# TravisDai/DLRM-FlexFlow

Hardware: AMD Instinct MI355X
Metric: samples/sec DLRM (MLPerf-like) at 1/2/4/8 MI355X; SOAP speedup vs pure DP (higher is better)
Workload: dtype fp32; 1 GPU; global_batch=8192, seq_len=1, parallelism=dp1, tables_rows=187767399, embedding_dim=128, interaction=dot, hip_graph=True, backend=none, process_world=1, fp32_gemm=bf16x3-split-big+native-f32-mfma, gemm_tuned_entries=21, gemm_staging=lds-dma

## Files before the change

csrc/bindings/hip_ops.cpp:

```cpp
#include <torch/extension.h>
#include <ATen/hip/HIPContext.h>
#include <cstring>
#include <vector>

extern "C" {
void fm_sgd_update_segs(float* W, float* G, float* V, unsigned short* Wc, const float* lr, const long* off,
                        const long* len, int nseg, float wd, float mom, int nesterov, int zero_g, hipStream_t s);
void fm_image_normalize(const unsigned char* src, void* dst, long N, int H, int W, const float* mean, const float* stdv,
                        int bf16, hipStream_t s);
int fm_gemm_dw_sgd(const void* A, long lda, const void* B, long ldb, float* W, long ldw, unsigned short* Wc, float* V,
                   const float* lr, float wd, float mom, int nesterov, int M, int N, int K, float* ws, long ws_bytes,
                   float* rowsum_a, int cfg, hipStream_t stream);
int fm_gemm_f32_dw_sgd(const float* A, long lda, const float* B, long ldb, float* W, long ldw, unsigned short* Wc,
                       float* V, const float* lr, float wd, float mom, int nesterov, int M, int N, int K, float* ws,
                       long ws_bytes, float* rowsum_a, int cfg, hipStream_t stream);
int fm_gemm(const void* A, long lda, long sA, int a_kcontig, const void* B, long ldb, long sB, int b_kcontig, void* C,
            long ldc, long sC, int c_fp32, const float* bias, int M, int N, int K, int batch, float alpha, int beta,
            int act, float* ws, long ws_bytes, int ksplit_req, const void* act_y, long lday, int bwd_act,
            float* colsum, float* rowsum_a, hipStream_t stream);
void fm_gemm_f32_set_split(int on);
void fm_gemm_set_dma(int on);
int fm_gemm_dma_enabled();
void fm_embedding_set_bwd_mode(int count);
int fm_gemm_f32_get_split();
// ... 9 lines not shown
                        int nesterov, int bf16, hipStream_t s);
void fm_skinny_fwd_f32_launch(const float* x, long ldx, const float* w, const float* bias, float* y, long ldy, long B, int K,
                              int act, hipStream_t s);
void fm_skinny_bwd_f32_launch(const float* x, long ldx, const float* w, const float* y, long ldy, const float* dy, long lddy,
                              float* dx, long lddx, int dx_acc, float* dw, float* db, long B, int K, int act, int bact,
                              hipStream_t s);
void fm_skinny_fwd(const void* x, long ldx, const void* w, const float* bias, void* y, long ldy, long B, int K, int act,
                   hipStream_t s);
void fm_skinny_bwd(const void* x, long ldx, const void* w, const void* y, long ldy, const void* dy, long lddy, void* dx,
                   long lddx, int dx_acc, float* dw, float* db, long B, int K, int act, int bact, hipStream_t s);
void fm_init_fill(float* out, long rows, long cols, long r0, long c0, long ldg, int kind, unsigned seed, float a, float b,
                  hipStream_t s);
void fm_embedding_fwd(const void* idx, int idx64, const float* W, void* out, int out_bf16, long B, int bag, int rows, int D,
                      long ldo, float scale, hipStream_t s);
void fm_embedding_bwd(const void* idx, int idx64, const void* dy, int dy_bf16, float* W, const float* lr, long B, int bag,
                      int rows, int D, long ldg, float scale, hipStream_t s);
void fm_embedding_fwd_multi(int n, const float* const* W, const void* const* idx, const int* idx64, void* const* out,
                            const long* ldo, const long* lo, const int* rows, const int* D, const int* bag,
                            const float* scale, int out_bf16, long B, hipStream_t st);
void fm_embedding_bwd_multi(int n, float* const* W, const void* const* idx, const int* idx64, const void* const* dy,
                            const long* ldg, const long* lo, const int* rows, const int* D, const int* bag,
                            const float* scale, int dy_bf16, const float* lr, long B, int* const* owner,
                            int* const* dups, int* const* ndup, hipStream_t st);
void fm_sdp_coalesce(int n, const void* const* idx, const int* idx64, const void* const* dy, const long* ldg,
                     const long* lo, const int* rows, const int* D, const int* bag, const float* scale, int dy_bf16, long B,
                     int* const* slot, int* const* cid, int* const* ids, float* const* g, int* const* count, hipStream_t st);
void fm_sdp_apply_segments(int n, int segs, int own_seg, float* const* W, const int* D, const int* const* seg_ids,
                           const float* const* seg_g, const int* const* seg_count, int* const* slot, int* const* own_count,
                           const int* nmax, const float* lr, hipStream_t st);
void fm_emb_adagrad_apply(int n, float* const* W, float* const* H, const int* D, const int* const* ids,
                          const float* const* g, int* const* count, int* const* slot, const int* nmax, const float* lr,
                          float eps, hipStream_t st);
void fm_emb_rowwise_adagrad_apply(int n, float* const* W, float* const* h, const int* D, const int* const* ids,
                                  const float* const* g, int* const* count, int* const* slot, const int* nmax,
                                  const float* lr, float eps, hipStream_t st);
void fm_sdp_rowwise_merge_segments(int n, int segs, const int* rows, const int* D, const int* const* seg_ids,
                                   const float* const* seg_g, const int* const* seg_count, const int* const* own_ids,
                                   int* const* own_count, int* const* slot, int* const* mids, float* const* mg,
                                   int* const* mcount, const int* nmax, const int* mcap, hipStream_t st);
void fm_strided_copy4_run(const void* src, void* dst, int bf16, const int* d, const long* ss, const long* ts, long so,
                          long to, int acc, hipStream_t st);
void fm_dot_interaction_fwd(const void* const* z, int F, long ldz, void* out, long ldo, long B, int D, int W, int self,
                            hipStream_t s);
void fm_dot_interaction_bwd(const void* const* z, int F, long ldz, const void* dout, long ldo, void* const* dz, long lddz,
                            unsigned acc_mask, long B, int D, int self, hipStream_t s);
void fm_dot_interaction_fwd_f32(const float* const* z, int F, long ldz, float* out, long ldo, long B, int D, int W, int self,
// ... 388 lines not shown
  bool any = false;
  if (claim.has_value()) {
    TORCH_CHECK(claim->size() == 3 * W.size(), "claim: 3 buffers per table");
    for (size_t k = 0; k < W.size(); ++k) {
      const auto& o = (*claim)[3 * k];
      if (!o.has_value() || !o->defined()) continue;
      const auto& d = (*claim)[3 * k + 1];
      const auto& c = (*claim)[3 * k + 2];
      TORCH_CHECK(o->scalar_type() == torch::kInt32 && o->numel() >= W[k].size(0), "claim owner: int32 [rows]");
      TORCH_CHECK(d.has_value() && d->scalar_type() == torch::kInt32 && d->numel() >= idx[k].numel(), "claim dups");
      TORCH_CHECK(c.has_value() && c->scalar_type() == torch::kInt32 && c->numel() >= 1, "claim ndup");
      own[k] = o->data_ptr<int>();
      dup[k] = d->data_ptr<int>();
      nd[k] = c->data_ptr<int>();
      any = true;
    }
  }
  fm_embedding_bwd_multi((int)W.size(), a.Wm.data(), a.idx.data(), a.idx64.data(), a.cact.data(), a.ld.data(), lo.data(),
                         a.rows.data(), a.D.data(), a.bag.data(), a.scale.data(), is_bf16(dy[0]),
                         lr.has_value() && lr->defined() ? lr->data_ptr<float>() : nullptr, a.B,
                         any ? own.data() : nullptr, any ? dup.data() : nullptr, any ? nd.data() : nullptr, cur());
}

void sdp_coalesce(std::vector<torch::Tensor> W, std::vector<torch::Tensor> idx, std::vector<torch::Tensor> dy,
                  std::vector<int64_t> ldg, std::vector<double> scale, std::vector<int64_t> row_lo,
                  std::vector<torch::Tensor> slot, std::vector<torch::Tensor> cid, std::vector<torch::Tensor> ids,
                  std::vector<torch::Tensor> g, std::vector<torch::Tensor> count) {
  if (W.empty()) return;
  TabArgs a = tab_args(W, idx, dy, ldg, scale);
  std::vector<long> lo = row_offsets(row_lo, W.size());
  const size_t n = W.size();
  TORCH_CHECK(slot.size() == n && cid.size() == n && ids.size() == n && g.size() == n && count.size() == n,
              "sdp_coalesce: one buffer of each kind per table");
  std::vector<int*> ps, pc, pi, pn;
  std::vector<float*> pg;
  for (size_t k = 0; k < n; ++k) {
    TORCH_CHECK(slot[k].scalar_type() == torch::kInt32 && slot[k].numel() >= W[k].size(0), "sdp slot: int32 [rows]");
    TORCH_CHECK(cid[k].scalar_type() == torch::kInt32 && cid[k].numel() >= idx[k].numel(), "sdp cid: int32 [B*bag]");
    TORCH_CHECK(ids[k].scalar_type() == torch::kInt32 && ids[k].numel() >= idx[k].numel(), "sdp ids: int32 [B*bag]");
    TORCH_CHECK(g[k].scalar_type() == torch::kFloat32 && g[k].numel() >= idx[k].numel() * W[k].size(1),
                "sdp g: fp32 [B*bag, D]");
    TORCH_CHECK(count[k].scalar_type() == torch::kInt32 && count[k].numel() >= 1, "sdp count: int32 [1]");
    ps.push_back(slot[k].data_ptr<int>());
    pc.push_back(cid[k].data_ptr<int>());
    pi.push_back(ids[k].data_ptr<int>());
    pg.push_back(g[k].data_ptr<float>());
// ... 869 lines not shown
  m.def("cnhwc_wprep", &cnhwc_wprep);
  m.def("conv_nhwc_fwd", &conv_nhwc_fwd);
  m.def("conv_nhwc_dgrad", &conv_nhwc_dgrad);
  m.def("gemm_f32_set_split", [](int mode) { fm_gemm_f32_set_split(mode); });
  m.def("gemm_set_dma", [](int on) { fm_gemm_set_dma(on); });
  m.def("gemm_dma_enabled", []() { return fm_gemm_dma_enabled(); });
  m.def("gemm_f32_get_split", []() { return fm_gemm_f32_get_split(); });
  m.def("embedding_set_bwd_mode", [](bool count) { fm_embedding_set_bwd_mode(count ? 1 : 0); });
  m.def("conv_nhwc_dgrad_strided", &conv_nhwc_dgrad_strided);
  m.def("conv_nhwc_wgrad", &conv_nhwc_wgrad);
  m.def("conv_s2d", &conv_s2d);
  m.def("stem_supported", &stem_supported);
  m.def("stem_wgrad_ws", &stem_wgrad_ws);
  m.def("stem_wf_elems", &stem_wf_elems);
  m.def("stem_fwd", &stem_fwd);
  m.def("stem_wgrad", &stem_wgrad);
  m.def("conv_w_s2d", &conv_w_s2d);
  m.def("embedding_fwd", &embedding_fwd);
  m.def("embedding_bwd", &embedding_bwd);
  m.def("embedding_fwd_multi", &embedding_fwd_multi, py::arg("W"), py::arg("idx"), py::arg("out"), py::arg("ldo"),
        py::arg("scale"), py::arg("row_lo") = std::vector<int64_t>{});
  m.def("embedding_bwd_multi", &embedding_bwd_multi, py::arg("W"), py::arg("idx"), py::arg("dy"), py::arg("ldg"),
        py::arg("scale"), py::arg("lr"), py::arg("claim"), py::arg("row_lo") = std::vector<int64_t>{});
  m.def("strided_copy4", &strided_copy4);
  m.def("sdp_coalesce", &sdp_coalesce);
  m.def("sdp_apply", &sdp_apply);
  m.def("emb_adagrad_apply", &emb_adagrad_apply);
  m.def("emb_rowwise_adagrad_apply", &emb_rowwise_adagrad_apply);
  m.def("sdp_rowwise_merge", &sdp_rowwise_merge);
  m.def("dot_fwd", &dot_fwd);
  m.def("dot_bwd", &dot_bwd, py::arg("zs"), py::arg("ldz"), py::arg("dout"), py::arg("ldo"), py::arg("dzs"),
        py::arg("lddz"), py::arg("acc_mask"), py::arg("D"), py::arg("self"), py::arg("act0") = 10);
  m.def("sgd", &sgd);
  m.def("adam", &adam);
  m.def("adagrad", &adagrad);
  m.def("cast_bf16", &cast_bf16);
  m.def("loss", &loss, py::arg("loss_type"), py::arg("logits"), py::arg("labels"), py::arg("grad"), py::arg("scale"),
        py::arg("acc"), py::arg("mask"), py::arg("clamp_t") = 0.0);
  m.def("unary_fwd", &unary_fwd);
  m.def("unary_bwd", &unary_bwd);
  m.def("binary_fwd", &binary_fwd);
  m.def("binary_bwd", &binary_bwd);
  m.def("act_bwd_bias", &act_bwd_bias);
  m.def("multi_copy", &multi_copy);
  m.def("image_normalize", &image_normalize);
  m.def("permute", &permute);
// ... 18 lines not shown
```

csrc/cpu/cpu_ops.cc:

```cpp
#include <torch/extension.h>
#include <ATen/Parallel.h>

#include <algorithm>
#include <cstdint>

#include "emb_kernels.h"

namespace {

void use_aten_pool() {
  static const bool done = [] {
    flexmi::cpu::set_parallel_for([](int64_t n, int64_t grain, int64_t max_threads,
                                     const std::function<void(int64_t, int64_t)>& fn) {
      if (max_threads > 0 && max_threads <= n) grain = std::max<int64_t>(grain, (n + max_threads - 1) / max_threads);
      at::parallel_for(0, n, grain, [&](int64_t b, int64_t e) { fn(b, e); });
    });
    return true;
  }();
  (void)done;
}

void check(const torch::Tensor& W, const torch::Tensor& idx, const torch::Tensor& rowt, const char* what) {
  TORCH_CHECK(W.device().is_cpu() && idx.device().is_cpu() && rowt.device().is_cpu(), what, ": CPU tensors");
  TORCH_CHECK(W.scalar_type() == torch::kFloat32 && W.dim() == 2 && W.is_contiguous(), what, ": contiguous fp32 table [R,D]");
  TORCH_CHECK(idx.dim() == 2 && idx.is_contiguous() &&
                  (idx.scalar_type() == torch::kInt32 || idx.scalar_type() == torch::kInt64), what,
              ": contiguous int32/int64 indices [B,bag]");
  TORCH_CHECK(rowt.scalar_type() == torch::kFloat32 && rowt.dim() == 2 && rowt.size(0) == idx.size(0) &&
// ... 6 lines not shown
  if (idx.scalar_type() == torch::kInt32)
    flexmi::cpu::embedding_bag_forward<int32_t>(W.data_ptr<float>(), W.size(0), W.size(1), idx.data_ptr<int32_t>(),
                                                idx.size(0), idx.size(1), row_lo, (float)scale, out.data_ptr<float>(),
                                                out.stride(0));
  else
    flexmi::cpu::embedding_bag_forward<int64_t>(W.data_ptr<float>(), W.size(0), W.size(1), idx.data_ptr<int64_t>(),
                                                idx.size(0), idx.size(1), row_lo, (float)scale, out.data_ptr<float>(),
                                                out.stride(0));
}

void embedding_bwd(torch::Tensor target, torch::Tensor idx, torch::Tensor dy, int64_t row_lo, double alpha) {
  check(target, idx, dy, "embedding_bwd");
  use_aten_pool();
  const int64_t B = idx.size(0), bag = idx.size(1), D = target.size(1);
  const int workers = (int)std::max<int64_t>(1, std::min<int64_t>(at::get_num_threads(), (B * bag * D) / 16384 + 1));
  if (idx.scalar_type() == torch::kInt32)
    flexmi::cpu::embedding_bag_backward<int32_t>(target.data_ptr<float>(), target.size(0), D, idx.data_ptr<int32_t>(), B,
                                                 bag, row_lo, dy.data_ptr<float>(), dy.stride(0), (float)alpha, workers);
  else
    flexmi::cpu::embedding_bag_backward<int64_t>(target.data_ptr<float>(), target.size(0), D, idx.data_ptr<int64_t>(), B,
                                                 bag, row_lo, dy.data_ptr<float>(), dy.stride(0), (float)alpha, workers);
}

bool avx2() { return flexmi::cpu::has_avx2(); }

}

void register_init_metrics(pybind11::module& m);

PYBIND11_MODULE(_cpu, m) {
  m.doc() = "flexmi native CPU kernels (embedding bag forward / backward / fused sparse SGD, counter-based init, loss + metrics)";
  m.def("embedding_fwd", &embedding_fwd, "out = scale * bag-sum of table rows");
  m.def("embedding_bwd", &embedding_bwd, "table rows += alpha * dy (dense grad or fused SGD)");
  m.def("avx2", &avx2);
  register_init_metrics(m);
}
```

csrc/cpu/emb_kernels.cc:

```cpp
#include "emb_kernels.h"

#include <immintrin.h>

#include <algorithm>
#include <thread>
#include <vector>

namespace flexmi {
namespace cpu {

namespace {

ParallelFor g_pf;

void default_parallel_for(int64_t n, int64_t grain, int64_t max_threads, const std::function<void(int64_t, int64_t)>& fn) {
  const int64_t hw = std::max<int64_t>(1, (int64_t)std::thread::hardware_concurrency());
  const int64_t nt = std::max<int64_t>(1, std::min<int64_t>({hw, max_threads > 0 ? max_threads : hw, (n + grain - 1) / grain}));
  if (nt <= 1) {
    fn(0, n);
    return;
  }
  std::vector<std::thread> th;
  const int64_t per = (n + nt - 1) / nt;
  for (int64_t t = 0; t < nt; ++t) {
// ... 91 lines not shown
  pfor(B, std::max<int64_t>(1, 2048 / std::max<int64_t>(1, D * bag / 64)), 0, [&](int64_t b0, int64_t b1) {
    for (int64_t b = b0; b < b1; ++b) {
      if (avx) bag_avx2<I>(W, rows, D, idx + b * bag, bag, row_lo, scale, out + b * ld_out);
      else bag_scalar<I>(W, rows, D, idx + b * bag, bag, row_lo, scale, out + b * ld_out);
    }
  });
}

template <typename I>
void embedding_bag_backward(float* target, int64_t rows, int64_t D, const I* idx, int64_t B, int64_t bag, int64_t row_lo,
                            const float* dy, int64_t ld_dy, float alpha, int workers) {
  const int64_t nw = std::max<int64_t>(1, workers > 0 ? workers : (B * bag * D) / 16384 + 1);
  pfor(nw, 1, nw, [&](int64_t p0, int64_t p1) {
    for (int64_t p = p0; p < p1; ++p)
      for (int64_t b = 0; b < B; ++b)
        for (int64_t j = 0; j < bag; ++j) {
          const int64_t r = (int64_t)idx[b * bag + j] - row_lo;
          if (r < 0 || r >= rows || r % nw != p) continue;
          axpy(target + r * D, dy + b * ld_dy, alpha, D);
        }
  });
}

template void embedding_bag_forward<int32_t>(const float*, int64_t, int64_t, const int32_t*, int64_t, int64_t, int64_t, float,
                                             float*, int64_t);
template void embedding_bag_forward<int64_t>(const float*, int64_t, int64_t, const int64_t*, int64_t, int64_t, int64_t, float,
                                             float*, int64_t);
template void embedding_bag_backward<int32_t>(float*, int64_t, int64_t, const int32_t*, int64_t, int64_t, int64_t,
                                              const float*, int64_t, float, int);
template void embedding_bag_backward<int64_t>(float*, int64_t, int64_t, const int64_t*, int64_t, int64_t, int64_t,
                                              const float*, int64_t, float, int);

}
}
```

csrc/cpu/emb_kernels.h:

```cpp
#pragma once
#include <cstdint>
#include <functional>

namespace flexmi {
namespace cpu {

using ParallelFor = std::function<void(int64_t, int64_t, int64_t, const std::function<void(int64_t, int64_t)>&)>;
void set_parallel_for(ParallelFor pf);

bool has_avx2();

template <typename I>
void embedding_bag_forward(const float* W, int64_t rows, int64_t D, const I* idx, int64_t B, int64_t bag, int64_t row_lo,
                           float scale, float* out, int64_t ld_out);

template <typename I>
void embedding_bag_backward(float* target, int64_t rows, int64_t D, const I* idx, int64_t B, int64_t bag, int64_t row_lo,
                            const float* dy, int64_t ld_dy, float alpha, int workers);

}
}
```

csrc/kernels/embedding.hip:

```cpp
#include "common.h"

#include <algorithm>
#include <cstdlib>
#include <cstring>
#include <vector>

namespace {

constexpr int MAXT = 32;
constexpr int TINY_ROWS = 16;

struct TabDesc {
  const float* W;
  const void* idx;
  void* act;
  long ld;
  long lo;
  int rows, D, bag;
  float scale;
};

FM_DEVICE long local_row(long r, long lo, int rows, bool& ok) {
  const long l = r - lo;
  ok = (unsigned long)l < (unsigned long)rows;
// ... 425 lines not shown

template <bool I64>
void launch_bwd(const TabSet& s, int m, bool tiny, bool dy_bf16, const float* lr, long B, int maxD, hipStream_t st) {
  if (tiny) {
    size_t lds = 0;
    for (int i = 0; i < m; ++i) lds = std::max(lds, (size_t)s.t[i].rows * s.t[i].D * 4 * 4);
    static bool attr = false;
    if (!attr) {
      (void)hipFuncSetAttribute((const void*)fm_emb_bwd_tiny_multi<unsigned short, I64>,
                                hipFuncAttributeMaxDynamicSharedMemorySize, 160 << 10);
      (void)hipFuncSetAttribute((const void*)fm_emb_bwd_tiny_multi<float, I64>,
                                hipFuncAttributeMaxDynamicSharedMemorySize, 160 << 10);
      attr = true;
    }
    const int chunk = B <= 16384 ? 64 : B <= 32768 ? 128 : 256;
    dim3 grid((unsigned)((B + chunk - 1) / chunk), m);
    if (dy_bf16) hipLaunchKernelGGL((fm_emb_bwd_tiny_multi<unsigned short, I64>), grid, dim3(256), lds, st, s, lr, B, chunk);
    else hipLaunchKernelGGL((fm_emb_bwd_tiny_multi<float, I64>), grid, dim3(256), lds, st, s, lr, B, chunk);
  } else {
    const int rpi = std::max(1, 256 / std::min(256, maxD));
    dim3 grid((unsigned)std::max<long>(1, emb_bwd_cap(std::min<long>((B + rpi - 1) / rpi, 2048))), m);
    if (dy_bf16) hipLaunchKernelGGL((fm_emb_bwd_atomic_multi<unsigned short, I64>), grid, dim3(256), 0, st, s, lr, B);
    else hipLaunchKernelGGL((fm_emb_bwd_atomic_multi<float, I64>), grid, dim3(256), 0, st, s, lr, B);
  }
}

struct SdpDesc {
  const void* idx;
  const void* dy;
  long ld;
  long lo;
  int rows, D, bag;
  float scale;
  int* slot;
  int* cid;
  int* ids;
  float* g;
  int* count;
};
struct SdpSet {
  SdpDesc t[MAXT];
  int n;
};

template <bool I64>
__global__ void __launch_bounds__(256) fm_sdp_claim(SdpSet s, long B) {
// ... 393 lines not shown
    for (int k = 0; k < n; ++k) {
      if (claimable(k)) continue;
      if (kind_of(k) == kind && (idx64[k] != 0) == wide) sel.push_back(k);
    }
    for (size_t base = 0; base < sel.size(); base += MAXT) {
      TabSet s;
      int m = (int)std::min<size_t>(MAXT, sel.size() - base);
      int maxD = 1;
      for (int i = 0; i < m; ++i) {
        int k = sel[base + i];
        s.t[i] = TabDesc{W[k], idx[k], const_cast<void*>(dy[k]), ldg[k], lo ? lo[k] : 0, rows[k], D[k], bag[k], scale[k]};
        maxD = std::max(maxD, D[k]);
      }
      s.n = m;
      if (wide) {
        launch_bwd<true>(s, m, tiny, dy_bf16, lr, B, maxD, st);
      } else {
        launch_bwd<false>(s, m, tiny, dy_bf16, lr, B, maxD, st);
      }
    }
  }
}

extern "C" void fm_embedding_fwd(const void* idx, int idx64, const float* W, void* out, int out_bf16, long B, int bag,
                                 int rows, int D, long ldo, float scale, hipStream_t s) {
  fm_embedding_fwd_multi(1, &W, &idx, &idx64, &out, &ldo, nullptr, &rows, &D, &bag, &scale, out_bf16, B, s);
}

extern "C" void fm_embedding_bwd(const void* idx, int idx64, const void* dy, int dy_bf16, float* W, const float* lr,
                                 long B, int bag, int rows, int D, long ldg, float scale, hipStream_t s) {
  fm_embedding_bwd_multi(1, &W, &idx, &idx64, &dy, &ldg, nullptr, &rows, &D, &bag, &scale, dy_bf16, lr, B, nullptr,
                         nullptr, nullptr, s);
}

extern "C" void fm_sdp_coalesce(int n, const void* const* idx, const int* idx64, const void* const* dy, const long* ldg,
                                const long* lo, const int* rows, const int* D, const int* bag, const float* scale,
                                int dy_bf16, long B, int* const* slot, int* const* cid, int* const* ids, float* const* g,
                                int* const* count, hipStream_t st) {
  if (B <= 0 || n <= 0) return;
  for (int wide = 0; wide < 2; ++wide) {
    std::vector<int> sel;
    for (int k = 0; k < n; ++k)
      if ((idx64[k] != 0) == (wide != 0)) sel.push_back(k);
    for (size_t base = 0; base < sel.size(); base += MAXT) {
      SdpSet s;
      const int m = (int)std::min<size_t>(MAXT, sel.size() - base);
// ... 138 lines not shown
```

flexmi/ops/embedding.py:

```python
from __future__ import annotations

import math
import os

import torch

from flexmi.core.initializers import UniformInitializer
from flexmi.core.types import AggrMode, DataType, OperatorType
from flexmi.parallel.layout import Layout

from .base import Op, OpCtx, store
from . import _kernels as K



NATIVE_CPU = os.environ.get("FM_CPU_NATIVE", "1") != "0"
_CPU_MOD = []


def _cpu_ext():
    if not _CPU_MOD:
        try:
            from flexmi import _cpu as m
        except ImportError:
# ... 218 lines not shown
            bag = idx.shape[1]
            li, ok = self._local_rows(idx, self._row_lo(ctx), dw.shape[0])
            dw.index_add_(0, li.reshape(-1), g.repeat_interleave(bag, dim=0) * ok.reshape(-1, 1).to(g.dtype))

    @staticmethod
    def can_group(a, b, ca, cb):
        return (ca.outputs[0].dtype == cb.outputs[0].dtype and a.sparse_sgd == b.sparse_sgd
                and getattr(a, "sparse_adagrad", None) == getattr(b, "sparse_adagrad", None)
                and getattr(a, "sparse_rowwise", None) == getattr(b, "sparse_rowwise", None)
                and getattr(a, "sparse_dp", None) == getattr(b, "sparse_dp", None)
                and ca.inputs[0].shape[0] == cb.inputs[0].shape[0])

    @staticmethod
    def forward_group(ops, ctxs):
        if not ctxs[0].hip:
            for op, c in zip(ops, ctxs):
                op.forward(c)
            return
        K.C().embedding_fwd_multi([c.weights[0] for c in ctxs], [c.inputs[0] for c in ctxs],
                                  [c.outputs[0] for c in ctxs], [c.outputs[0].stride(0) for c in ctxs],
                                  [1.0 / c.inputs[0].shape[1] if op.aggr == AggrMode.AGGR_MODE_AVG else 1.0
                                   for op, c in zip(ops, ctxs)],
                                  [Embedding._row_lo(c) for c in ctxs])

    @staticmethod
    def backward_group(ops, ctxs):
        if not ctxs[0].hip:
            for op, c in zip(ops, ctxs):
                op.backward(c)
            return
        if ops[0].sparse_adagrad is not None:
            Embedding.adagrad_group(ops, ctxs)
            return
        if ops[0].sparse_rowwise is not None:
            Embedding.rowwise_group(ops, ctxs)
            return
        scales = [1.0 / c.inputs[0].shape[1] if op.aggr == AggrMode.AGGR_MODE_AVG else 1.0 for op, c in zip(ops, ctxs)]
        if ops[0].sparse_sgd:
            tables = [c.weights[0] for c in ctxs]
            lr = ctxs[0].lr
        else:
            tables = [c.weight_grads[0] for c in ctxs]
            lr = None
        claim = None
        if ops[0].sparse_sgd:
            bufs = [op._claim_buffers(c) for op, c in zip(ops, ctxs)]
            if any(b is not None for b in bufs):
                claim = []
                for b in bufs:
                    claim.extend(b if b is not None else (None, None, None))
        K.C().embedding_bwd_multi(tables, [c.inputs[0] for c in ctxs], [c.out_grads[0] for c in ctxs],
                                  [c.out_grads[0].stride(0) for c in ctxs], scales, lr, claim,
                                  [Embedding._row_lo(c) for c in ctxs])

    @staticmethod
    def sdp_state(ops, ctxs, holders, rank):
        c0 = ctxs[0]
        st = c0.saved.get("sdp")
        if st is None:
            cls = SparseRowwiseDPState if ops[0].sparse_rowwise is not None else SparseDPState
            st = cls(ops, ctxs, holders, rank)
            c0.saved["sdp"] = st
        return st

    @staticmethod
    def sdp_pack(ops, ctxs, st=None):
# ... 115 lines not shown
                                    [c.weights[0].shape[1] for c in ctxs], st.R)
            K.C().emb_rowwise_adagrad_apply([c.weights[0] for c in ctxs], H, st.mids, st.mg, st.mcount, st.slot, lr,
                                            Embedding._rowwise_eps(ops))
            return
        lrf = lr.to(torch.float32)
        for k, (op, c) in enumerate(zip(ops, ctxs)):
            w = c.weights[0]
            D = w.shape[1]
            ns = [int(st.rcount[s][k].item()) for s in range(st.R)]
            if not sum(ns):
                continue
            uniq, inv = torch.unique(torch.cat([st.rids[s][k][:ns[s]].long() for s in range(st.R)]), return_inverse=True)
            summed = torch.zeros((uniq.numel(), D), dtype=torch.float32)
            o = 0
            for s in range(st.R):
                summed.index_add_(0, inv[o:o + ns[s]], st.rg[s][k][:ns[s] * D].view(ns[s], D))
                o += ns[s]
            Embedding._rowwise_rule(w, H[k], uniq, summed, lrf, float(op.sparse_rowwise))

    CLAIM = True
    CLAIM_RATIO = 0.2
    COUNT = False
    TINY_ROWS = 64

    def _claim_buffers(self, ctx):
        if not Embedding.CLAIM:
            return None
        s = ctx.saved
        if "claim" not in s:
            w, idx = ctx.weights[0], ctx.inputs[0]
            big = w.shape[0] > (Embedding.TINY_ROWS if Embedding.COUNT else Embedding.CLAIM_RATIO * idx.numel())
            if big and self.out_dim % 4 == 0:
                dev = w.device
                s["claim"] = (torch.full((w.shape[0],), -1, dtype=torch.int32, device=dev),
                              torch.empty(idx.numel(), dtype=torch.int32, device=dev),
                              torch.zeros(1, dtype=torch.int32, device=dev))
            else:
                s["claim"] = None
        return s["claim"]

    def flops(self, in_shapes, out_shapes):
        return float(in_shapes[0][0] * in_shapes[0][1] * out_shapes[0][1])

    @staticmethod
    def sdp_payload_words(lookups, D):
        return 1 + lookups * (1 + D)
# ... 12 lines not shown
```

Baseline: 7.100 million samples/s.

## Add bucketed update plan for sparse-SGD embedding backward built during forward

Adds a plan kernel that runs after the embedding forward. It counting-sorts each table's lookups into row-hash buckets and emits chunked work items. The backward then uses a planned kernel that gives each row a single accumulate-and-write, replacing the atomic scatter with claim buffers. Building the plan in forward is meant to take the sorting off the backward critical path and to reduce atomic contention on hot rows. The cost is an extra kernel launch, extra buffers, and a quadratic in-chunk dedup for buckets that hold multiple rows. It only applies to tables with at most 32768 lookups, which at batch 8192 means bag sizes up to 4.

```diff
diff --git a/csrc/bindings/hip_ops.cpp b/csrc/bindings/hip_ops.cpp
--- a/csrc/bindings/hip_ops.cpp
+++ b/csrc/bindings/hip_ops.cpp
@@ -55,6 +55,13 @@
                             const long* ldg, const long* lo, const int* rows, const int* D, const int* bag,
                             const float* scale, int dy_bf16, const float* lr, long B, int* const* owner,
                             int* const* dups, int* const* ndup, hipStream_t st);
+void fm_embedding_plan_multi(int n, const void* const* idx, const int* idx64, const long* lo, const int* rows,
+                             const int* bag, long B, int* const* order, int* const* orow, int* const* items,
+                             int* const* nitems, hipStream_t st);
+void fm_embedding_bwd_planned_multi(int n, float* const* W, const void* const* dy, const long* ldg, const int* rows,
+                                    const int* D, const int* bag, const float* scale, int dy_bf16, const float* lr, long B,
+                                    const int* const* order, const int* const* orow, const int* const* items,
+                                    const int* const* nitems, int waves_per_cu, hipStream_t st);
 void fm_sdp_coalesce(int n, const void* const* idx, const int* idx64, const void* const* dy, const long* ldg,
                      const long* lo, const int* rows, const int* D, const int* bag, const float* scale, int dy_bf16, long B,
                      int* const* slot, int* const* cid, int* const* ids, float* const* g, int* const* count, hipStream_t st);
@@ -489,6 +496,80 @@
                          any ? own.data() : nullptr, any ? dup.data() : nullptr, any ? nd.data() : nullptr, cur());
 }
 
+struct PlanBufs {
+  std::vector<int*> order, orow, items, nitems;
+};
+
+PlanBufs plan_bufs(const std::vector<torch::Tensor>& order, const std::vector<torch::Tensor>& orow,
+                   const std::vector<torch::Tensor>& items, const std::vector<torch::Tensor>& nitems,
+                   const std::vector<int64_t>& lookups) {
+  const size_t n = lookups.size();
+  TORCH_CHECK(order.size() == n && orow.size() == n && items.size() == n && nitems.size() == n, "plan: list sizes");
+  PlanBufs p;
+  for (size_t k = 0; k < n; ++k) {
+    for (const torch::Tensor* t : {&order[k], &orow[k], &items[k], &nitems[k]}) {
+      check_cuda(*t, "plan buffer");
+      TORCH_CHECK(t->scalar_type() == torch::kInt32 && t->is_contiguous(), "plan buffers: contiguous int32");
+    }
+    TORCH_CHECK(lookups[k] < (1L << 24), "plan: at most 2^24 lookups per table");
+    TORCH_CHECK(order[k].numel() >= lookups[k] && orow[k].numel() >= lookups[k] && items[k].numel() >= lookups[k] &&
+                    nitems[k].numel() >= 1, "plan buffers: one slot per lookup");
+    p.order.push_back(order[k].data_ptr<int>());
+    p.orow.push_back(orow[k].data_ptr<int>());
+    p.items.push_back(items[k].data_ptr<int>());
+    p.nitems.push_back(nitems[k].data_ptr<int>());
+  }
+  return p;
+}
+
+void embedding_plan_multi(std::vector<torch::Tensor> idx, std::vector<int64_t> rows, std::vector<int64_t> row_lo,
+                          std::vector<torch::Tensor> order, std::vector<torch::Tensor> orow,
+                          std::vector<torch::Tensor> items, std::vector<torch::Tensor> nitems) {
+  const size_t n = idx.size();
+  if (n == 0) return;
+  TORCH_CHECK(rows.size() == n, "embedding_plan_multi: list sizes");
+  std::vector<long> lo = row_offsets(row_lo, n);
+  std::vector<const void*> ip;
+  std::vector<int> i64, r, bag;
+  std::vector<int64_t> lookups;
+  const long B = idx[0].size(0);
+  for (size_t k = 0; k < n; ++k) {
+    check_cuda(idx[k], "idx");
+    TORCH_CHECK(idx[k].dim() == 2 && idx[k].is_contiguous() && idx[k].size(0) == B, "idx [B, bag], same batch");
+    TORCH_CHECK(idx[k].scalar_type() == torch::kInt32 || idx[k].scalar_type() == torch::kInt64, "idx int32/int64");
+    TORCH_CHECK(rows[k] >= 1 && rows[k] <= INT32_MAX, "rows");
+    ip.push_back(idx[k].data_ptr());
+    i64.push_back(idx[k].scalar_type() == torch::kInt64);
+    r.push_back((int)rows[k]);
+    bag.push_back((int)idx[k].size(1));
+    lookups.push_back(idx[k].numel());
+  }
+  PlanBufs p = plan_bufs(order, orow, items, nitems, lookups);
+  fm_embedding_plan_multi((int)n, ip.data(), i64.data(), lo.data(), r.data(), bag.data(), B, p.order.data(), p.orow.data(),
+                          p.items.data(), p.nitems.data(), cur());
+}
+
+void embedding_bwd_planned_multi(std::vector<torch::Tensor> W, std::vector<torch::Tensor> idx, std::vector<torch::Tensor> dy,
+                                 std::vector<int64_t> ldg, std::vector<double> scale, torch::Tensor lr,
+                                 std::vector<torch::Tensor> order, std::vector<torch::Tensor> orow,
+                                 std::vector<torch::Tensor> items, std::vector<torch::Tensor> nitems, int64_t waves_per_cu) {
+  if (W.empty()) return;
+  TabArgs a = tab_args(W, idx, dy, ldg, scale);
+  check_cuda(lr, "lr");
+  std::vector<int64_t> lookups;
+  for (size_t k = 0; k < W.size(); ++k) {
+    TORCH_CHECK(a.D[k] % 4 == 0 && a.D[k] <= 256 && ldg[k] % 4 == 0, "planned update: D % 4 == 0, D <= 256, ldg % 4 == 0");
+    TORCH_CHECK(dy[k].scalar_type() == dy[0].scalar_type(), "planned update: one gradient dtype");
+    lookups.push_back(idx[k].numel());
+  }
+  PlanBufs p = plan_bufs(order, orow, items, nitems, lookups);
+  std::vector<const int*> po(p.order.begin(), p.order.end()), pr(p.orow.begin(), p.orow.end()),
+      pi(p.items.begin(), p.items.end()), pn(p.nitems.begin(), p.nitems.end());
+  fm_embedding_bwd_planned_multi((int)W.size(), a.Wm.data(), a.cact.data(), a.ld.data(), a.rows.data(), a.D.data(),
+                                 a.bag.data(), a.scale.data(), is_bf16(dy[0]), lr.data_ptr<float>(), a.B, po.data(),
+                                 pr.data(), pi.data(), pn.data(), (int)waves_per_cu, cur());
+}
+
 void sdp_coalesce(std::vector<torch::Tensor> W, std::vector<torch::Tensor> idx, std::vector<torch::Tensor> dy,
                   std::vector<int64_t> ldg, std::vector<double> scale, std::vector<int64_t> row_lo,
                   std::vector<torch::Tensor> slot, std::vector<torch::Tensor> cid, std::vector<torch::Tensor> ids,
@@ -1404,6 +1485,11 @@
         py::arg("scale"), py::arg("row_lo") = std::vector<int64_t>{});
   m.def("embedding_bwd_multi", &embedding_bwd_multi, py::arg("W"), py::arg("idx"), py::arg("dy"), py::arg("ldg"),
         py::arg("scale"), py::arg("lr"), py::arg("claim"), py::arg("row_lo") = std::vector<int64_t>{});
+  m.def("embedding_plan_multi", &embedding_plan_multi, py::arg("idx"), py::arg("rows"), py::arg("row_lo"),
+        py::arg("order"), py::arg("orow"), py::arg("items"), py::arg("nitems"));
+  m.def("embedding_bwd_planned_multi", &embedding_bwd_planned_multi, py::arg("W"), py::arg("idx"), py::arg("dy"),
+        py::arg("ldg"), py::arg("scale"), py::arg("lr"), py::arg("order"), py::arg("orow"), py::arg("items"),
+        py::arg("nitems"), py::arg("waves_per_cu") = 16);
   m.def("strided_copy4", &strided_copy4);
   m.def("sdp_coalesce", &sdp_coalesce);
   m.def("sdp_apply", &sdp_apply);
diff --git a/csrc/cpu/cpu_ops.cc b/csrc/cpu/cpu_ops.cc
--- a/csrc/cpu/cpu_ops.cc
+++ b/csrc/cpu/cpu_ops.cc
@@ -3,7 +3,10 @@
 
 #include <algorithm>
 #include <cstdint>
+#include <tuple>
+#include <vector>
 
+#include "../kernels/emb_plan.h"
 #include "emb_kernels.h"
 
 namespace {
@@ -56,6 +59,48 @@
                                                  bag, row_lo, dy.data_ptr<float>(), dy.stride(0), (float)alpha, workers);
 }
 
+std::tuple<torch::Tensor, torch::Tensor, torch::Tensor> embedding_plan(torch::Tensor idx, int64_t rows, int64_t row_lo) {
+  TORCH_CHECK(idx.device().is_cpu() && idx.is_contiguous() &&
+                  (idx.scalar_type() == torch::kInt32 || idx.scalar_type() == torch::kInt64),
+              "embedding_plan: contiguous int32/int64 CPU indices");
+  TORCH_CHECK(rows >= 1 && idx.numel() < fm_plan::kMaxEntries, "embedding_plan: rows >= 1, fewer than 2^24 lookups");
+  const int64_t n = idx.numel();
+  torch::Tensor order = torch::empty({n}, torch::kInt32), orow = torch::empty({n}, torch::kInt32);
+  std::vector<uint32_t> packed((size_t)n);
+  const int64_t k = idx.scalar_type() == torch::kInt32
+                        ? flexmi::cpu::embedding_plan<int32_t>(idx.data_ptr<int32_t>(), n, rows, row_lo, order.data_ptr<int32_t>(),
+                                                               orow.data_ptr<int32_t>(), packed.data())
+                        : flexmi::cpu::embedding_plan<int64_t>(idx.data_ptr<int64_t>(), n, rows, row_lo, order.data_ptr<int32_t>(),
+                                                               orow.data_ptr<int32_t>(), packed.data());
+  torch::Tensor items = torch::empty({k, 3}, torch::kInt64);
+  int64_t* ip = items.data_ptr<int64_t>();
+  int64_t used = 0;
+  for (int64_t i = 0; i < k; ++i) {
+    ip[3 * i] = fm_plan::item_start(packed[i]);
+    ip[3 * i + 1] = fm_plan::item_len(packed[i]);
+    ip[3 * i + 2] = fm_plan::item_multi(packed[i]) ? 1 : 0;
+    used += ip[3 * i + 1];
+  }
+  return {order.narrow(0, 0, used), orow.narrow(0, 0, used), items};
+}
+
+torch::Tensor plan_unpack_items(torch::Tensor packed) {
+  TORCH_CHECK(packed.device().is_cpu() && packed.scalar_type() == torch::kInt32 && packed.is_contiguous(), "packed int32");
+  const int64_t k = packed.numel();
+  torch::Tensor items = torch::empty({k, 3}, torch::kInt64);
+  int64_t* ip = items.data_ptr<int64_t>();
+  const int32_t* pp = packed.data_ptr<int32_t>();
+  for (int64_t i = 0; i < k; ++i) {
+    const uint32_t v = (uint32_t)pp[i];
+    ip[3 * i] = fm_plan::item_start(v);
+    ip[3 * i + 1] = fm_plan::item_len(v);
+    ip[3 * i + 2] = fm_plan::item_multi(v) ? 1 : 0;
+  }
+  return items;
+}
+
+int64_t plan_bucket(int64_t local_row, int64_t rows) { return fm_plan::bucket_of(local_row, fm_plan::num_buckets(rows)); }
+
 bool avx2() { return flexmi::cpu::has_avx2(); }
 
 }
@@ -66,6 +111,11 @@
   m.doc() = "flexmi native CPU kernels (embedding bag forward / backward / fused sparse SGD, counter-based init, loss + metrics)";
   m.def("embedding_fwd", &embedding_fwd, "out = scale * bag-sum of table rows");
   m.def("embedding_bwd", &embedding_bwd, "table rows += alpha * dy (dense grad or fused SGD)");
+  m.def("embedding_plan", &embedding_plan, "host reference of the GPU update plan: (order, orow, items[k,3])");
+  m.def("plan_unpack_items", &plan_unpack_items, "packed plan items -> [k,3] (start, len, multi)");
+  m.def("plan_bucket", &plan_bucket, "bucket of a local row in a table of `rows` rows");
+  m.attr("PLAN_CHUNK") = fm_plan::kChunk;
+  m.attr("PLAN_MAX_BUCKETS") = fm_plan::kMaxBuckets;
   m.def("avx2", &avx2);
   register_init_metrics(m);
 }
diff --git a/csrc/cpu/emb_kernels.cc b/csrc/cpu/emb_kernels.cc
--- a/csrc/cpu/emb_kernels.cc
+++ b/csrc/cpu/emb_kernels.cc
@@ -1,4 +1,6 @@
 #include "emb_kernels.h"
+
+#include "../kernels/emb_plan.h"
 
 #include <immintrin.h>
 
@@ -137,6 +139,37 @@
   });
 }
 
+template <typename I>
+int64_t embedding_plan(const I* idx, int64_t n, int64_t rows, int64_t row_lo, int32_t* order, int32_t* orow,
+                       uint32_t* items) {
+  const int nb = fm_plan::num_buckets(rows);
+  std::vector<int64_t> at(nb + 1, 0);
+  auto local = [&](int64_t e) { return (int64_t)idx[e] - row_lo; };
+  for (int64_t e = 0; e < n; ++e) {
+    const int64_t r = local(e);
+    if (r >= 0 && r < rows) ++at[fm_plan::bucket_of(r, nb) + 1];
+  }
+  for (int b = 0; b < nb; ++b) at[b + 1] += at[b];
+  std::vector<int64_t> cur(at.begin(), at.end() - 1);
+  for (int64_t e = 0; e < n; ++e) {
+    const int64_t r = local(e);
+    if (r < 0 || r >= rows) continue;
+    const int64_t p = cur[fm_plan::bucket_of(r, nb)]++;
+    order[p] = (int32_t)e;
+    orow[p] = (int32_t)r;
+  }
+  int64_t k = 0;
+  for (int b = 0; b < nb; ++b) {
+    const int64_t c = at[b + 1] - at[b];
+    for (int64_t o = 0; o < c; o += fm_plan::kChunk)
+      items[k++] = fm_plan::pack_item((uint32_t)(at[b] + o), (int)std::min<int64_t>(fm_plan::kChunk, c - o),
+                                      c > fm_plan::kChunk);
+  }
+  return k;
+}
+
+template int64_t embedding_plan<int32_t>(const int32_t*, int64_t, int64_t, int64_t, int32_t*, int32_t*, uint32_t*);
+template int64_t embedding_plan<int64_t>(const int64_t*, int64_t, int64_t, int64_t, int32_t*, int32_t*, uint32_t*);
 template void embedding_bag_forward<int32_t>(const float*, int64_t, int64_t, const int32_t*, int64_t, int64_t, int64_t, float,
                                              float*, int64_t);
 template void embedding_bag_forward<int64_t>(const float*, int64_t, int64_t, const int64_t*, int64_t, int64_t, int64_t, float,
diff --git a/csrc/cpu/emb_kernels.h b/csrc/cpu/emb_kernels.h
--- a/csrc/cpu/emb_kernels.h
+++ b/csrc/cpu/emb_kernels.h
@@ -18,5 +18,9 @@
 void embedding_bag_backward(float* target, int64_t rows, int64_t D, const I* idx, int64_t B, int64_t bag, int64_t row_lo,
                             const float* dy, int64_t ld_dy, float alpha, int workers);
 
+template <typename I>
+int64_t embedding_plan(const I* idx, int64_t n, int64_t rows, int64_t row_lo, int32_t* order, int32_t* orow,
+                       uint32_t* items);
+
 }
 }
diff --git a/csrc/kernels/emb_plan.h b/csrc/kernels/emb_plan.h
--- /dev/null
+++ b/csrc/kernels/emb_plan.h
@@ -0,0 +1,32 @@
+#pragma once
+#include <cstdint>
+
+#if defined(__HIPCC__)
+#define FM_PLAN_HD __host__ __device__ inline
+#else
+#define FM_PLAN_HD inline
+#endif
+
+namespace fm_plan {
+
+constexpr int kMaxBuckets = 8192;
+constexpr int kChunk = 32;
+constexpr int kItemLenBits = 7;
+constexpr long kMaxEntries = 1L << 24;
+
+FM_PLAN_HD int num_buckets(long rows) { return rows < kMaxBuckets ? (int)rows : kMaxBuckets; }
+
+FM_PLAN_HD int bucket_of(long local_row, int nb) {
+  return nb == kMaxBuckets ? (int)(local_row & (kMaxBuckets - 1)) : (int)local_row;
+}
+
+FM_PLAN_HD int items_of(int count) { return (count + kChunk - 1) / kChunk; }
+
+FM_PLAN_HD uint32_t pack_item(uint32_t start, int len, bool multi) {
+  return start << (kItemLenBits + 1) | (uint32_t)(len - 1) << 1 | (multi ? 1u : 0u);
+}
+FM_PLAN_HD uint32_t item_start(uint32_t it) { return it >> (kItemLenBits + 1); }
+FM_PLAN_HD int item_len(uint32_t it) { return (int)((it >> 1) & ((1u << kItemLenBits) - 1)) + 1; }
+FM_PLAN_HD bool item_multi(uint32_t it) { return (it & 1u) != 0; }
+
+}
diff --git a/csrc/kernels/embedding.hip b/csrc/kernels/embedding.hip
--- a/csrc/kernels/embedding.hip
+++ b/csrc/kernels/embedding.hip
@@ -1,4 +1,5 @@
 #include "common.h"
+#include "emb_plan.h"
 
 #include <algorithm>
 #include <cstdlib>
@@ -471,6 +472,260 @@
     dim3 grid((unsigned)std::max<long>(1, emb_bwd_cap(std::min<long>((B + rpi - 1) / rpi, 2048))), m);
     if (dy_bf16) hipLaunchKernelGGL((fm_emb_bwd_atomic_multi<unsigned short, I64>), grid, dim3(256), 0, st, s, lr, B);
     else hipLaunchKernelGGL((fm_emb_bwd_atomic_multi<float, I64>), grid, dim3(256), 0, st, s, lr, B);
+  }
+}
+
+struct PlanDesc {
+  const void* idx;
+  long lo;
+  int rows, bag;
+  int* order;
+  int* orow;
+  uint32_t* items;
+  int* nitems;
+};
+struct PlanSet {
+  PlanDesc t[MAXT];
+  int n;
+};
+
+constexpr int PLAN_THREADS = 1024;
+constexpr int PLAN_PER = fm_plan::kMaxBuckets / PLAN_THREADS;
+constexpr int PLAN_EB = 8;
+
+FM_DEVICE int plan_block_scan(int v, int* wsum, int& total) {
+  const int lane = threadIdx.x & 63, wave = threadIdx.x >> 6;
+  int x = v;
+#pragma unroll
+  for (int off = 1; off < 64; off <<= 1) {
+    const int y = __shfl_up(x, off, 64);
+    if (lane >= off) x += y;
+  }
+  if (lane == 63) wsum[wave] = x;
+  __syncthreads();
+  int base = 0, tot = 0;
+#pragma unroll
+  for (int w = 0; w < PLAN_THREADS / 64; ++w) {
+    const int sw = wsum[w];
+    if (w < wave) base += sw;
+    tot += sw;
+  }
+  __syncthreads();
+  total = tot;
+  return base + x - v;
+}
+
+template <bool I64>
+__global__ void __launch_bounds__(PLAN_THREADS) fm_emb_plan_multi(PlanSet s, long B) {
+  __shared__ int cnt[fm_plan::kMaxBuckets];
+  __shared__ int wsum[PLAN_THREADS / 64];
+  const PlanDesc& d = s.t[blockIdx.x];
+  const int nb = fm_plan::num_buckets(d.rows);
+  const long n = B * d.bag;
+  const int tid = threadIdx.x;
+  for (int i = tid; i < fm_plan::kMaxBuckets; i += PLAN_THREADS) cnt[i] = 0;
+  __syncthreads();
+  for (long base = tid; base - tid < n; base += (long)PLAN_THREADS * PLAN_EB) {
+    long r[PLAN_EB];
+    bool ok[PLAN_EB];
+#pragma unroll
+    for (int u = 0; u < PLAN_EB; ++u) {
+      const long e = base + (long)u * PLAN_THREADS;
+      r[u] = local_row(ldi<I64>(d.idx, min(e, n - 1)), d.lo, d.rows, ok[u]);
+      ok[u] = ok[u] && e < n;
+    }
+#pragma unroll
+    for (int u = 0; u < PLAN_EB; ++u)
+      if (ok[u]) atomicAdd(&cnt[fm_plan::bucket_of(r[u], nb)], 1);
+  }
+  __syncthreads();
+  int c[PLAN_PER], mine = 0, total;
+#pragma unroll
+  for (int j = 0; j < PLAN_PER; ++j) {
+    c[j] = cnt[tid * PLAN_PER + j];
+    mine += c[j];
+  }
+  int at = plan_block_scan(mine, wsum, total);
+#pragma unroll
+  for (int j = 0; j < PLAN_PER; ++j) {
+    cnt[tid * PLAN_PER + j] = at;
+    at += c[j];
+  }
+  __syncthreads();
+  for (long base = tid; base - tid < n; base += (long)PLAN_THREADS * PLAN_EB) {
+    long r[PLAN_EB];
+    bool ok[PLAN_EB];
+#pragma unroll
+    for (int u = 0; u < PLAN_EB; ++u) {
+      const long e = base + (long)u * PLAN_THREADS;
+      r[u] = local_row(ldi<I64>(d.idx, min(e, n - 1)), d.lo, d.rows, ok[u]);
+      ok[u] = ok[u] && e < n;
+    }
+#pragma unroll
+    for (int u = 0; u < PLAN_EB; ++u)
+      if (ok[u]) {
+        const int p = atomicAdd(&cnt[fm_plan::bucket_of(r[u], nb)], 1);
+        d.order[p] = (int)(base + (long)u * PLAN_THREADS);
+        d.orow[p] = (int)r[u];
+      }
+  }
+  __syncthreads();
+  int first = tid == 0 ? 0 : cnt[tid * PLAN_PER - 1], ni = 0;
+  int end[PLAN_PER];
+#pragma unroll
+  for (int j = 0; j < PLAN_PER; ++j) {
+    end[j] = cnt[tid * PLAN_PER + j];
+    ni += fm_plan::items_of(end[j] - (j ? end[j - 1] : first));
+  }
+  int k = plan_block_scan(ni, wsum, total);
+#pragma unroll
+  for (int j = 0; j < PLAN_PER; ++j) {
+    const int b0 = j ? end[j - 1] : first, cb = end[j] - b0;
+    for (int o = 0; o < cb; o += fm_plan::kChunk)
+      d.items[k++] = fm_plan::pack_item((uint32_t)(b0 + o), min(fm_plan::kChunk, cb - o), cb > fm_plan::kChunk);
+  }
+  if (tid == 0) *d.nitems = total;
+}
+
+struct ApplyDesc {
+  float* W;
+  const void* dy;
+  long ld;
+  int D, bag;
+  float scale;
+  int uniform;
+  int cap;
+  const int* order;
+  const int* orow;
+  const uint32_t* items;
+  const int* nitems;
+};
+struct ApplySet {
+  ApplyDesc t[MAXT];
+  int n;
+};
+
+template <typename GT>
+FM_DEVICE f32x4_t plan_ldg(const GT* p) {
+  if constexpr (sizeof(GT) == 2) {
+    const bf16x4_t g = *reinterpret_cast<const bf16x4_t*>(p);
+    return f32x4_t{bf2f((unsigned short)g[0]), bf2f((unsigned short)g[1]), bf2f((unsigned short)g[2]),
+                   bf2f((unsigned short)g[3])};
+  } else {
+    return *reinterpret_cast<const f32x4_t*>(p);
+  }
+}
+
+FM_DEVICE void plan_write(float* wr, int c, int lc, int lpr, f32x4_t acc, float mul, bool multi) {
+  if (!multi) {
+    f32x4_t* wp = reinterpret_cast<f32x4_t*>(wr + c);
+    *wp = *wp + mul * acc;
+    return;
+  }
+  if ((64 % lpr) == 0) {
+    const int gb = (int)(threadIdx.x & 63) - lc;
+#pragma unroll
+    for (int q = 0; q < 4; ++q) {
+      const int col = lc + q * lpr, src = gb + (col >> 2), j = col & 3;
+      const float t0 = __shfl(acc[0], src, 64), t1 = __shfl(acc[1], src, 64);
+      const float t2 = __shfl(acc[2], src, 64), t3 = __shfl(acc[3], src, 64);
+      atomicAdd(wr + col, mul * (j == 0 ? t0 : j == 1 ? t1 : j == 2 ? t2 : t3));
+    }
+  } else {
+#pragma unroll
+    for (int j = 0; j < 4; ++j) atomicAdd(wr + c + j, mul * acc[j]);
+  }
+}
+
+template <typename GT>
+__global__ void __launch_bounds__(256) fm_emb_bwd_planned_multi(ApplySet s, const float* __restrict__ lr) {
+  constexpr int U = 4;
+  const ApplyDesc& d = s.t[blockIdx.y];
+  const float mul = -lr[0] * d.scale;
+  const int lpr = d.D >> 2;
+  const int rpi = 256 / lpr;
+  const int sub = threadIdx.x / lpr, lc = threadIdx.x - sub * lpr;
+  if (sub >= rpi) return;
+  const int c = lc * 4;
+  const int ni = min(*d.nitems, d.cap);
+  const int stride = (int)gridDim.x * rpi;
+  int it = (int)blockIdx.x * rpi + sub;
+  if (it >= ni) return;
+  const GT* dy = reinterpret_cast<const GT*>(d.dy);
+  const int bag = d.bag;
+  uint32_t cur = d.items[it];
+  uint32_t nxt = d.items[min(it + stride, ni - 1)];
+  int e[U], r[U];
+#pragma unroll
+  for (int u = 0; u < U; ++u) {
+    const int p = (int)fm_plan::item_start(cur) + min(u, fm_plan::item_len(cur) - 1);
+    e[u] = d.order[p];
+    r[u] = d.orow[p];
+  }
+  for (; it < ni; it += stride) {
+    const int start = (int)fm_plan::item_start(cur), len = fm_plan::item_len(cur);
+    const bool multi = fm_plan::item_multi(cur);
+    f32x4_t g[U], w[U];
+#pragma unroll
+    for (int u = 0; u < U; ++u) g[u] = plan_ldg<GT>(dy + (long)(bag == 1 ? e[u] : e[u] / bag) * d.ld + c);
+#pragma unroll
+    for (int u = 0; u < U; ++u) w[u] = *reinterpret_cast<const f32x4_t*>(d.W + (long)r[u] * d.D + c);
+    int rc[U];
+#pragma unroll
+    for (int u = 0; u < U; ++u) rc[u] = r[u];
+    const uint32_t nn = d.items[min(it + 2 * stride, ni - 1)];
+#pragma unroll
+    for (int u = 0; u < U; ++u) {
+      const int p = (int)fm_plan::item_start(nxt) + min(u, fm_plan::item_len(nxt) - 1);
+      e[u] = d.order[p];
+      r[u] = d.orow[p];
+    }
+    cur = nxt;
+    nxt = nn;
+    if (!multi && len <= U) {
+#pragma unroll
+      for (int u = 0; u < U; ++u) {
+        bool lead = u < len;
+        f32x4_t sum = g[u];
+#pragma unroll
+        for (int v = 0; v < u; ++v) lead = lead && rc[v] != rc[u];
+#pragma unroll
+        for (int v = u + 1; v < U; ++v) {
+          const bool same = v < len && rc[v] == rc[u];
+          sum += same ? g[v] : f32x4_t{0.f, 0.f, 0.f, 0.f};
+        }
+        if (lead) *reinterpret_cast<f32x4_t*>(d.W + (long)rc[u] * d.D + c) = w[u] + mul * sum;
+      }
+    } else if (d.uniform) {
+      f32x4_t acc = {0.f, 0.f, 0.f, 0.f};
+#pragma unroll
+      for (int u = 0; u < U; ++u) acc += u < len ? g[u] : f32x4_t{0.f, 0.f, 0.f, 0.f};
+      for (int i = U; i < len; i += U) {
+        int eb[U];
+#pragma unroll
+        for (int u = 0; u < U; ++u) eb[u] = d.order[start + min(i + u, len - 1)];
+        f32x4_t gb[U];
+#pragma unroll
+        for (int u = 0; u < U; ++u) gb[u] = plan_ldg<GT>(dy + (long)(bag == 1 ? eb[u] : eb[u] / bag) * d.ld + c);
+#pragma unroll
+        for (int u = 0; u < U; ++u) acc += i + u < len ? gb[u] : f32x4_t{0.f, 0.f, 0.f, 0.f};
+      }
+      plan_write(d.W + (long)rc[0] * d.D, c, lc, lpr, acc, mul, multi);
+    } else {
+      for (int i = 0; i < len; ++i) {
+        const int ri = d.orow[start + i];
+        bool lead = true;
+        for (int v = 0; v < i; ++v) lead = lead && d.orow[start + v] != ri;
+        if (!lead) continue;
+        f32x4_t acc = {0.f, 0.f, 0.f, 0.f};
+        for (int v = i; v < len; ++v) {
+          const int ev = d.order[start + v];
+          const f32x4_t gv = plan_ldg<GT>(dy + (long)(bag == 1 ? ev : ev / bag) * d.ld + c);
+          if (d.orow[start + v] == ri) acc += gv;
+        }
+        plan_write(d.W + (long)ri * d.D, c, lc, lpr, acc, mul, multi);
+      }
+    }
   }
 }
 
@@ -910,6 +1165,60 @@
   }
 }
 
+extern "C" void fm_embedding_plan_multi(int n, const void* const* idx, const int* idx64, const long* lo, const int* rows,
+                                        const int* bag, long B, int* const* order, int* const* orow, int* const* items,
+                                        int* const* nitems, hipStream_t st) {
+  if (B <= 0) return;
+  for (int wide = 0; wide < 2; ++wide) {
+    std::vector<int> sel;
+    for (int k = 0; k < n; ++k)
+      if ((idx64[k] != 0) == (wide != 0)) sel.push_back(k);
+    for (size_t base = 0; base < sel.size(); base += MAXT) {
+      PlanSet s;
+      const int m = (int)std::min<size_t>(MAXT, sel.size() - base);
+      for (int i = 0; i < m; ++i) {
+        const int k = sel[base + i];
+        s.t[i] = PlanDesc{idx[k], lo ? lo[k] : 0, rows[k], bag[k], order[k], orow[k],
+                          reinterpret_cast<uint32_t*>(items[k]), nitems[k]};
+      }
+      s.n = m;
+      if (wide) hipLaunchKernelGGL((fm_emb_plan_multi<true>), dim3(m), dim3(PLAN_THREADS), 0, st, s, B);
+      else hipLaunchKernelGGL((fm_emb_plan_multi<false>), dim3(m), dim3(PLAN_THREADS), 0, st, s, B);
+    }
+  }
+}
+
+extern "C" void fm_embedding_bwd_planned_multi(int n, float* const* W, const void* const* dy, const long* ldg,
+                                               const int* rows, const int* D, const int* bag, const float* scale,
+                                               int dy_bf16, const float* lr, long B, const int* const* order,
+                                               const int* const* orow, const int* const* items,
+                                               const int* const* nitems, int waves_per_cu, hipStream_t st) {
+  if (B <= 0 || n <= 0) return;
+  static int cus = 0;
+  if (!cus) {
+    int dev = 0;
+    (void)hipGetDevice(&dev);
+    if (hipDeviceGetAttribute(&cus, hipDeviceAttributeMultiprocessorCount, dev) != hipSuccess || cus <= 0) cus = 256;
+  }
+  for (size_t base = 0; base < (size_t)n; base += MAXT) {
+    ApplySet s;
+    const int m = (int)std::min<size_t>(MAXT, n - base);
+    long most = 1;
+    for (int i = 0; i < m; ++i) {
+      const int k = (int)base + i;
+      const long cap = B * bag[k];
+      s.t[i] = ApplyDesc{W[k], dy[k], ldg[k], D[k], bag[k], scale[k], rows[k] <= fm_plan::kMaxBuckets ? 1 : 0, (int)cap,
+                         order[k], orow[k], reinterpret_cast<const uint32_t*>(items[k]), nitems[k]};
+      most = std::max(most, (cap + (256 / (D[k] / 4)) - 1) / (256 / (D[k] / 4)));
+    }
+    s.n = m;
+    const long want = std::max<long>(1, (long)cus * std::max(1, waves_per_cu) / 4 / m);
+    dim3 grid((unsigned)std::min(most, want), m);
+    if (dy_bf16) hipLaunchKernelGGL((fm_emb_bwd_planned_multi<unsigned short>), grid, dim3(256), 0, st, s, lr);
+    else hipLaunchKernelGGL((fm_emb_bwd_planned_multi<float>), grid, dim3(256), 0, st, s, lr);
+  }
+}
+
 extern "C" void fm_embedding_fwd(const void* idx, int idx64, const float* W, void* out, int out_bf16, long B, int bag,
                                  int rows, int D, long ldo, float scale, hipStream_t s) {
   fm_embedding_fwd_multi(1, &W, &idx, &idx64, &out, &ldo, nullptr, &rows, &D, &bag, &scale, out_bf16, B, s);
diff --git a/flexmi/ops/embedding.py b/flexmi/ops/embedding.py
--- a/flexmi/ops/embedding.py
+++ b/flexmi/ops/embedding.py
@@ -264,6 +264,32 @@
                                   [1.0 / c.inputs[0].shape[1] if op.aggr == AggrMode.AGGR_MODE_AVG else 1.0
                                    for op, c in zip(ops, ctxs)],
                                   [Embedding._row_lo(c) for c in ctxs])
+        if ops[0].sparse_sgd and ctxs[0].training:
+            Embedding._build_plans(ops, ctxs)
+
+    @staticmethod
+    def _build_plans(ops, ctxs, only_stale=False):
+        planned = []
+        for op, c in zip(ops, ctxs):
+            p = op._plan_buffers(c)
+            if p is not None:
+                planned.append((op, c, p))
+        todo = [(op, c, p) for op, c, p in planned
+                if not (only_stale and p["fresh"] and p["key"] == Embedding._plan_key(c))]
+        if todo:
+            K.C().embedding_plan_multi([c.inputs[0] for _, c, _ in todo], [c.weights[0].shape[0] for _, c, _ in todo],
+                                       [Embedding._row_lo(c) for _, c, _ in todo], [p["order"] for _, _, p in todo],
+                                       [p["orow"] for _, _, p in todo], [p["items"] for _, _, p in todo],
+                                       [p["nitems"] for _, _, p in todo])
+            for _, c, p in todo:
+                p["key"] = Embedding._plan_key(c)
+                p["fresh"] = True
+        return planned
+
+    @staticmethod
+    def _plan_key(ctx):
+        idx = ctx.inputs[0]
+        return (idx.data_ptr(), tuple(idx.shape), idx.dtype, Embedding._row_lo(ctx))
 
     @staticmethod
     def backward_group(ops, ctxs):
@@ -284,6 +310,25 @@
         else:
             tables = [c.weight_grads[0] for c in ctxs]
             lr = None
+        if ops[0].sparse_sgd:
+            cand = [(op, c) for op, c in zip(ops, ctxs) if c.out_grads[0].stride(0) % 4 == 0]
+            planned = Embedding._build_plans([op for op, _ in cand], [c for _, c in cand], only_stale=True)
+            if planned:
+                done = {id(c) for _, c, _ in planned}
+                pc = [c for _, c, _ in planned]
+                K.C().embedding_bwd_planned_multi([c.weights[0] for c in pc], [c.inputs[0] for c in pc],
+                                                  [c.out_grads[0] for c in pc], [c.out_grads[0].stride(0) for c in pc],
+                                                  [s for s, c in zip(scales, ctxs) if id(c) in done], lr,
+                                                  [p["order"] for _, _, p in planned], [p["orow"] for _, _, p in planned],
+                                                  [p["items"] for _, _, p in planned], [p["nitems"] for _, _, p in planned],
+                                                  Embedding.PLAN_WAVES)
+                for _, _, p in planned:
+                    p["fresh"] = False
+                keep = [k for k, c in enumerate(ctxs) if id(c) not in done]
+                if not keep:
+                    return
+                ops, ctxs = [ops[k] for k in keep], [ctxs[k] for k in keep]
+                tables, scales = [tables[k] for k in keep], [scales[k] for k in keep]
         claim = None
         if ops[0].sparse_sgd:
             bufs = [op._claim_buffers(c) for op, c in zip(ops, ctxs)]
@@ -445,6 +490,29 @@
     CLAIM_RATIO = 0.2
     COUNT = False
     TINY_ROWS = 64
+
+    PLAN = os.environ.get("FM_EMB_PLAN", "1") != "0"
+    PLAN_MAX_LOOKUPS = 32768
+    PLAN_WAVES = 16
+
+    def _plan_buffers(self, ctx):
+        if not (Embedding.PLAN and Embedding.CLAIM and not Embedding.COUNT and self.sparse_sgd and ctx.hip):
+            return None
+        w, idx = ctx.weights[0], ctx.inputs[0]
+        n = idx.numel()
+        if not (w.dtype == torch.float32 and w.dim() == 2 and w.shape[1] % 4 == 0 and w.shape[1] <= 256
+                and 0 < n <= Embedding.PLAN_MAX_LOOKUPS and idx.dim() == 2 and idx.is_contiguous()
+                and idx.dtype in (torch.int32, torch.int64)):
+            return None
+        p = ctx.saved.get("plan")
+        if p is None or p["order"].numel() < n:
+            dev = w.device
+            p = ctx.saved["plan"] = {"order": torch.empty(n, dtype=torch.int32, device=dev),
+                                     "orow": torch.empty(n, dtype=torch.int32, device=dev),
+                                     "items": torch.empty(n, dtype=torch.int32, device=dev),
+                                     "nitems": torch.zeros(1, dtype=torch.int32, device=dev),
+                                     "key": None, "fresh": False}
+        return p
 
     def _claim_buffers(self, ctx):
         if not Embedding.CLAIM:
```

After: 7.174 million samples/s (median of 6 runs). About the same (+1.0%).
